# parrot-tts/Parrot-TTS

Hardware: AMD Instinct MI355X
Metric: audio samples/sec (16 kHz; see config.note) + RTF, 256-unit batch-64 per GPU (higher is better)
Workload: dtype f32 (f16x3 split products)

## Files before the change

### parrot_tts_amd/build.py

```python
from __future__ import annotations

import os
import subprocess
import sys
from concurrent.futures import ThreadPoolExecutor

HERE = os.path.dirname(os.path.abspath(__file__))
CSRC = os.path.join(HERE, "csrc")
LIB = os.path.join(HERE, "libparrot_hip.so")
OBJ = os.path.join(HERE, "build")
SOURCES = sorted(f for f in os.listdir(CSRC) if f.endswith(".hip"))
HEADERS = sorted(f for f in os.listdir(CSRC) if f.endswith(".h")) + [os.path.join("..", "..", "include", h) for h in ("parrot_hip.h", "parrot_hip_debug.h")]
FLAGS = ["--offload-arch=gfx950", "-O3", "-std=c++17", "-fPIC"]
TU_FLAGS = {f: ["-mllvm", "-disable-machine-sink"] for f in ("tu_split16.hip", "tu_split16_wide.hip", "tu_split16_xpl.hip")}


def _stale() -> bool:
    if not os.path.exists(LIB):
        return True
    t = os.path.getmtime(LIB)
    return any(os.path.getmtime(os.path.join(CSRC, f)) > t for f in SOURCES + HEADERS)


def build(force: bool = False, verbose: bool = False, extra_flags=(), lib_path: str = None, obj_dir: str = None) -> str:
    if lib_path is None and not force and not _stale():
        return LIB
    hipcc = os.environ.get("HIPCC", "/opt/rocm/bin/hipcc")
    LIB_OUT, OBJ_OUT = lib_path or LIB, obj_dir or OBJ
    os.makedirs(OBJ_OUT, exist_ok=True)

    def compile_one(src):
        obj = os.path.join(OBJ_OUT, os.path.splitext(src)[0] + ".o")
        tu = [] if os.environ.get("PARROT_NO_TU_FLAGS") else TU_FLAGS.get(src, [])
        cmd = [hipcc] + FLAGS + tu + list(extra_flags) + ["-c", os.path.join(CSRC, src), "-o", obj]
        if verbose:
            print(" ".join(cmd), file=sys.stderr)
        subprocess.run(cmd, check=True, cwd=CSRC)
# ... 21 lines not shown
```

### parrot_tts_amd/csrc/conv_mfma.h

```cpp
#pragma once
#include <hip/hip_runtime.h>
#include <stdint.h>
#include <algorithm>

#include "conv_consts.h"

namespace parrot {

__host__ __device__ __forceinline__ int row_true_len(int n, int mul, int add) { return n > 0 ? n * mul + add : 0; }

struct DynLdsOnce {
    bool done[64] = {};
};
inline hipError_t ensure_dyn_lds(DynLdsOnce& st, const void* kern, size_t lds) {
    int dev = 0;
    hipError_t e = hipGetDevice(&dev);
    if (e != hipSuccess) return e;
    const bool tracked = dev >= 0 && dev < 64;
    if (tracked && st.done[dev]) return hipSuccess;
    e = hipFuncSetAttribute(kern, hipFuncAttributeMaxDynamicSharedMemorySize, (int)lds);
    if (e == hipSuccess && tracked) st.done[dev] = true;
    return e;
}


typedef float f32x16 __attribute__((ext_vector_type(16)));
typedef float f32x4 __attribute__((ext_vector_type(4)));

// ... 145 lines not shown
            const int mbase = m_wave + mt * 32 + 4 * half;
            const int o0 = mbase / p.u, rem0 = mbase - o0 * p.u;
#pragma unroll
            for (int nt = 0; nt < WN; ++nt) {
                const int n = n_wave + nt * 32 + l31;
#pragma unroll
                for (int r = 0; r < 16; ++r) {
                    const int cr = (r & 3) + 8 * (r >> 2);
                    const int rem = rem0 + cr;
                    const int dq = (rem * p.u_inv16) >> 16;
                    const int o = o0 + dq;
                    const int tau = n * p.u + (rem - dq * p.u);
                    const bool ok = (mbase + cr < p.M) && (n < p.Ncols) && (tau < p.Tout);
                    const float v = acc[mt][nt][r] + ((p.bias && ok) ? p.bias[o] : 0.f);
                    if (ok) yb[o * p.Tout + tau] = apply_act(v, p.act);
                }
            }
        }
        return;
    }
    const bool late_res = rb != nullptr && !fold_res;
    const bool has_acc = p.epi != EPI_STORE;
    const bool do_div = p.epi == EPI_ADD_DIV;
    const float act_lo = (p.act == ACT_RELU) ? 0.f : -INFINITY;
#pragma unroll
    for (int mt = 0; mt < WM; ++mt) {
        const int mbase = m_wave + mt * 32 + 4 * half;
#pragma unroll
        for (int nt = 0; nt < WN; ++nt) {
            const int n = n_wave + nt * 32 + l31;
            const bool colok = n < p.Ncols;
#pragma unroll
            for (int g = 0; g < 2; ++g) {
                int off[8];
                float rv[8], yv[8];
#pragma unroll
                for (int q = 0; q < 8; ++q) {
                    const int r = g * 8 + q;
                    const int m = mbase + (r & 3) + 8 * (r >> 2);
                    off[q] = (colok && m < p.M) ? m * p.Tout + n : -1;
                    rv[q] = 0.f;
                    yv[q] = 0.f;
                }
                if (late_res) {
#pragma unroll
                    for (int q = 0; q < 8; ++q) rv[q] = rb[off[q] < 0 ? 0 : off[q]];
                }
                if (has_acc) {
#pragma unroll
                    for (int q = 0; q < 8; ++q) yv[q] = yb[off[q] < 0 ? 0 : off[q]];
                }
                float v[8];
#pragma unroll
                for (int q = 0; q < 8; ++q) v[q] = yv[q] + (fmaxf(acc[mt][nt][g * 8 + q], act_lo) + rv[q]);
                if (do_div) {
#pragma unroll
                    for (int q = 0; q < 8; ++q) v[q] = v[q] / p.div;
                }
#pragma unroll
                for (int q = 0; q < 8; ++q)
                    if (off[q] >= 0) yb[off[q]] = v[q];
            }
        }
    }
}

struct RowTile {
    __amdgpu_buffer_rsrc_t rsrc;
};
__device__ __forceinline__ RowTile row_tile(const float* base, int rows, int row_elems) {
    const size_t a = reinterpret_cast<size_t>(base);
    const unsigned lo = __builtin_amdgcn_readfirstlane((unsigned)a), hi = __builtin_amdgcn_readfirstlane((unsigned)(a >> 32));
    RowTile t;
    t.rsrc = __builtin_amdgcn_make_buffer_rsrc(reinterpret_cast<void*>(((size_t)hi << 32) | lo), 0,
                                               __builtin_amdgcn_readfirstlane(rows * row_elems * 4), 0x00020000);
    return t;
}
__device__ __forceinline__ float row_tile_load(const RowTile& t, int voff, int soff) {
    return __builtin_bit_cast(float, __builtin_amdgcn_raw_buffer_load_b32(t.rsrc, voff, soff, 0));
}
__device__ __forceinline__ void row_tile_store(const RowTile& t, float v, int voff, int soff) {
// ... 34 lines not shown
        for (int r = 0; r < 16; ++r) bs[r] = p.bias ? p.bias[min(m0 + 4 * half + (r & 3) + 8 * (r >> 2), p.M - 1)] * p.acc_scale : 0.f;
        if (fold_res) {
#pragma unroll
            for (int nt = 0; nt < WN; ++nt)
#pragma unroll
                for (int r = 0; r < 16; ++r) acc[mt][nt][r] = fmaf(acc[mt][nt][r], p.acc_scale, bs[r]);
        } else {
#pragma unroll
            for (int nt = 0; nt < WN; ++nt)
#pragma unroll
                for (int r = 0; r < 16; ++r) acc[mt][nt][r] = bs[r];
        }
    }
}

template <int WM, int WN>
__device__ __forceinline__ void conv_epilogue_lean(const ConvParams& p, f32x16 (&acc)[WM][WN], int b, int m_wave, int n_wave, int half, int l31) {
    float* __restrict__ yb = p.y + (size_t)b * p.y_bstride;
    const float* __restrict__ rb = p.res ? p.res + (size_t)b * p.res_bstride : nullptr;
    const bool fold_res = rb != nullptr && p.act == ACT_NONE && p.fold_res != 0;
    const bool late_res = rb != nullptr && !fold_res;
    const bool has_acc = p.epi != EPI_STORE;
    const bool do_div = p.epi == EPI_ADD_DIV;
    const bool relu = p.act == ACT_RELU;
    const int row_bytes = p.Tout * 4;
    int vo[WN];
#pragma unroll
    for (int nt = 0; nt < WN; ++nt) {
        const int n = n_wave + nt * 32 + l31;
        vo[nt] = (n < p.Ncols) ? (4 * half * p.Tout + n) * 4 : (int)0x80000000;
    }
    const RowTile yt = row_tile(yb, p.M, p.Tout), rt = row_tile(late_res ? rb : yb, p.M, p.Tout);
#pragma unroll
    for (int mt = 0; mt < WM; ++mt) {
        const int m0 = m_wave + mt * 32;
#pragma unroll
        for (int nt = 0; nt < WN; ++nt) {
            float v[16];
#pragma unroll
            for (int r = 0; r < 16; ++r) v[r] = acc[mt][nt][r] * p.out_scale;
            if (relu) {
#pragma unroll
                for (int r = 0; r < 16; ++r) v[r] = fmaxf(v[r], 0.f);
            }
            if (late_res) {
                float rv[16];
#pragma unroll
                for (int r = 0; r < 16; ++r) rv[r] = row_tile_load(rt, vo[nt], (m0 + (r & 3) + 8 * (r >> 2)) * row_bytes);
#pragma unroll
                for (int r = 0; r < 16; ++r) v[r] = v[r] + rv[r];
            }
            if (has_acc) {
                float yv[16];
#pragma unroll
                for (int r = 0; r < 16; ++r) yv[r] = row_tile_load(yt, vo[nt], (m0 + (r & 3) + 8 * (r >> 2)) * row_bytes);
#pragma unroll
                for (int r = 0; r < 16; ++r) v[r] = yv[r] + v[r];
                if (do_div) {
#pragma unroll
                    for (int r = 0; r < 16; ++r) v[r] = v[r] / p.div;
                }
            }
#pragma unroll
            for (int r = 0; r < 16; ++r) row_tile_store(yt, v[r], vo[nt], (m0 + (r & 3) + 8 * (r >> 2)) * row_bytes);
        }
    }
}

template <int WAVES_M, int WAVES_N, int WM, int WN, int CI, int MINW>
__global__ __launch_bounds__(WAVES_M* WAVES_N * 64, MINW) void conv_mfma_kernel(const ConvParams p) {
    constexpr int NW = WAVES_M * WAVES_N;
    constexpr int BM = WAVES_M * WM * 32;
    constexpr int BN = WAVES_N * WN * 32;
    constexpr int RS = BN + CONV_HALO;
    constexpr int QN = CI / 8;
    constexpr int ROWS_PW = CI / NW;
    constexpr int COLS_IT = (RS + 63) / 64;
    static_assert(CI % 8 == 0 && CI % NW == 0, "CI must be a multiple of 8 and of the wave count");

    extern __shared__ __attribute__((aligned(16))) float smem[];

    const int tid = threadIdx.x;
    const int lane = tid & 63;
    const int wave = __builtin_amdgcn_readfirstlane(tid >> 6);
// ... 156 lines not shown
```

### parrot_tts_amd/csrc/conv_mfma16.h

```cpp
#pragma once
#include "conv_mfma.h"

namespace parrot {

template <int NT16, int MINW>
__global__ __launch_bounds__(256, MINW) void conv_mfma16_kernel(const ConvParams p) {
    constexpr int WCOLS = NT16 * 16;
    constexpr int BN = 4 * WCOLS;
    constexpr int RS = BN + CONV_HALO + 16;
    constexpr int CI = 16;
    constexpr int ROWS_PW = CI / 4;
    constexpr int COLS_IT = (RS + 63) / 64;
    static_assert(RS % 32 == 16, "row stride must be 16 mod 32 dwords");

    extern __shared__ __attribute__((aligned(16))) float smem[];

    const int tid = threadIdx.x;
    const int lane = tid & 63;
    const int wave = __builtin_amdgcn_readfirstlane(tid >> 6);
    const int kg = lane >> 4;
    const int l15 = lane & 15;

    const int b = blockIdx.x / p.tiles_n;
    const int tn = blockIdx.x - b * p.tiles_n;
// ... 82 lines not shown
#pragma unroll
            for (int e = 0; e < 4; ++e)
#pragma unroll
                for (int nt = 0; nt < NT16; ++nt) bv_nxt[e][nt] = xn[(4 * e) * RS + nt * 16];
            __builtin_amdgcn_sched_barrier(0);
#pragma unroll
            for (int e = 0; e < 4; ++e)
#pragma unroll
                for (int nt = 0; nt < NT16; ++nt)
                    acc[nt] = __builtin_amdgcn_mfma_f32_16x16x4f32(a_cur[e], bv_cur[e][nt], acc[nt], 0, 0, 0);
            __builtin_amdgcn_sched_barrier(0);
#pragma unroll
            for (int e = 0; e < 4; ++e)
#pragma unroll
                for (int nt = 0; nt < NT16; ++nt) bv_cur[e][nt] = bv_nxt[e][nt];
        }
        if (more) store_slab((c + 1) & 1);
        __syncthreads();
    }

    const bool late_res = rb != nullptr && !fold_res;
    const bool has_acc = p.epi != EPI_STORE;
    const bool do_div = p.epi == EPI_ADD_DIV;
    const float act_lo = (p.act == ACT_RELU) ? 0.f : -INFINITY;
#pragma unroll
    for (int nt = 0; nt < NT16; ++nt) {
        const int n = n_wave + nt * 16 + l15;
        int off[4];
        float rv[4], yv[4], v[4];
#pragma unroll
        for (int r = 0; r < 4; ++r) {
            const int m = 4 * kg + r;
            off[r] = (n < p.Ncols && m < p.M) ? m * p.Tout + n : -1;
            rv[r] = 0.f;
            yv[r] = 0.f;
        }
        if (late_res) {
#pragma unroll
            for (int r = 0; r < 4; ++r) rv[r] = rb[off[r] < 0 ? 0 : off[r]];
        }
        if (has_acc) {
#pragma unroll
            for (int r = 0; r < 4; ++r) yv[r] = yb[off[r] < 0 ? 0 : off[r]];
        }
#pragma unroll
        for (int r = 0; r < 4; ++r) v[r] = yv[r] + (fmaxf(acc[nt][r], act_lo) + rv[r]);
        if (do_div) {
#pragma unroll
            for (int r = 0; r < 4; ++r) v[r] = v[r] / p.div;
        }
#pragma unroll
        for (int r = 0; r < 4; ++r)
            if (off[r] >= 0) yb[off[r]] = v[r];
    }
}

constexpr int MFMA16_NT16 = 8;
inline hipError_t launch_conv_mfma16(const ConvParams& p, hipStream_t s) {
    constexpr int BN = 4 * MFMA16_NT16 * 16;
    const size_t lds = (size_t)2 * 16 * (BN + CONV_HALO + 16) * sizeof(float);
    auto kern = conv_mfma16_kernel<MFMA16_NT16, 2>;
    static DynLdsOnce lds_once;
    {
        hipError_t e = ensure_dyn_lds(lds_once, reinterpret_cast<const void*>(kern), (size_t)lds);
        if (e != hipSuccess) return e;
    }
    hipLaunchKernelGGL(kern, dim3(p.tiles_n * p.B), dim3(256), lds, s, p);
    return hipGetLastError();
}

}
```

### parrot_tts_amd/csrc/conv_split16.h

```cpp
#pragma once
#include "conv_split.h"

#ifndef PARROT_XPL_DMA
#define PARROT_XPL_DMA 1
#endif

namespace parrot {

template <class SCH, int WAVES_M, int WAVES_N, int TM, int TN, int K, int MINW = 2, bool XPL = false>
__global__ __launch_bounds__(WAVES_M* WAVES_N * 64, MINW) void conv_split16_kernel(const ConvParams p) {
    static_assert(K > 0, "tap count is a template parameter");
    constexpr int NPC = SCH::NP, NTERM = SCH::NT;
    constexpr int NW = WAVES_M * WAVES_N, NT = NW * 64;
    constexpr int BM = WAVES_M * TM * 16, BN = WAVES_N * TN * 16;
    constexpr int COLS = (BN + CONV_HALO + 63) / 64 * 64;
    constexpr int OCT_BYTES = COLS * 16, PIECE_BYTES = 4 * OCT_BYTES, BUF_BYTES = NPC * PIECE_BYTES;
    constexpr int LIVE = COLS * 4;
    constexpr int ITEMS = (LIVE + NT - 1) / NT;
    constexpr int STEP_BYTES = NPC * 1024;
    static_assert(LIVE % NT == 0, "every thread stages the same number of items");

    extern __shared__ __attribute__((aligned(16))) char smem_raw[];

    const int tid = threadIdx.x;
// ... 174 lines not shown
#pragma unroll
                        for (int i = 0; i < NPC; ++i) __builtin_amdgcn_sched_group_barrier(0x100, 1, 0);
                    } else if (slab_left > 0) {
                        __builtin_amdgcn_sched_group_barrier(0x020, 1, 0);
                        --slab_left;
                    }
                }
#pragma unroll
                for (int i = 0; i < NPC; ++i) __builtin_amdgcn_sched_group_barrier(0x020, 1, 0);
            }
        }
        __builtin_amdgcn_sched_barrier(0);
        if (more) store_slab((c + 1) & 1);
        if constexpr (XPL && PARROT_XPL_DMA) asm volatile("s_waitcnt vmcnt(%0)" ::"n"(TM * NPC) : "memory");
        __syncthreads();
    }

    float* __restrict__ yb = p.y + (size_t)b * p.y_bstride;
    const float* __restrict__ rb = p.res ? p.res + (size_t)b * p.res_bstride : nullptr;
    const int out_row_bytes = p.Tout * 4;
    const bool late_res = rb != nullptr;
    const bool has_acc = p.epi != EPI_STORE;
    const bool do_div = p.epi == EPI_ADD_DIV;
    const bool relu = p.act == ACT_RELU;
    const RowTile yt = row_tile(yb, p.M, p.Tout), rt = row_tile(late_res ? rb : yb, p.M, p.Tout);
    if (p.yplane) {
        int vo[TN];
#pragma unroll
        for (int tn = 0; tn < TN; ++tn) {
            const int n = n_wave + tn * 16 + l15;
            vo[tn] = (n < p.Ncols) ? (4 * g4 * p.Tout + n) * 4 : (int)0x80000000;
        }
#pragma unroll
        for (int tm = 0; tm < TM; ++tm) {
            const int m0 = m_wave + tm * 16;
            float rv[TN][4];
            if (late_res) {
#pragma unroll
                for (int tn = 0; tn < TN; ++tn)
#pragma unroll
                    for (int r = 0; r < 4; ++r) rv[tn][r] = row_tile_load(rt, vo[tn], (m0 + r) * out_row_bytes);
            }
#pragma unroll
            for (int tn = 0; tn < TN; ++tn)
#pragma unroll
                for (int r = 0; r < 4; ++r) {
// ... 59 lines not shown
#pragma unroll
        for (int tm = 0; tm < TM; ++tm) {
            const int m0 = m_wave + tm * 16;
            const int soff = m0 * out_row_bytes;
            f32x4 rv[TN], yv[TN];
            if (late_res) {
#pragma unroll
                for (int q = 0; q < TN; ++q) rv[q] = row_tile_load4(rt, vq[q], soff);
            }
            if (has_acc) {
#pragma unroll
                for (int q = 0; q < TN; ++q) yv[q] = row_tile_load4(yt, vq[q], soff);
            }
#pragma unroll
            for (int tn = 0; tn < TN; ++tn)
#pragma unroll
                for (int r = 0; r < 4; ++r) {
                    float v = acc[tm][tn][r] * p.out_scale;
                    if (relu) v = fmaxf(v, 0.f);
                    stg[wbase + r * RS + tn * 16] = v;
                }
#pragma unroll
            for (int q = 0; q < TN; ++q) {
                f32x4 v = *reinterpret_cast<const f32x4*>(stg + lq[q]);
                if (late_res) v = v + rv[q];
                if (has_acc) {
                    v = yv[q] + v;
                    if (do_div) v = v / p.div;
                }
                row_tile_store4(yt, v, vq[q], soff);
            }
        }
        return;
    }
    int vo[TN];
#pragma unroll
    for (int tn = 0; tn < TN; ++tn) {
        const int n = n_wave + tn * 16 + l15;
        vo[tn] = (n < p.Ncols) ? (4 * g4 * p.Tout + n) * 4 : (int)0x80000000;
    }
#pragma unroll
    for (int tm = 0; tm < TM; ++tm) {
        const int m0 = m_wave + tm * 16;
        float v[TN][4];
#pragma unroll
        for (int tn = 0; tn < TN; ++tn)
#pragma unroll
            for (int r = 0; r < 4; ++r) v[tn][r] = acc[tm][tn][r] * p.out_scale;
        if (relu) {
#pragma unroll
            for (int tn = 0; tn < TN; ++tn)
#pragma unroll
                for (int r = 0; r < 4; ++r) v[tn][r] = fmaxf(v[tn][r], 0.f);
// ... 1 lines not shown
        if (late_res) {
            float rv[TN][4];
#pragma unroll
            for (int tn = 0; tn < TN; ++tn)
#pragma unroll
                for (int r = 0; r < 4; ++r) rv[tn][r] = row_tile_load(rt, vo[tn], (m0 + r) * out_row_bytes);
#pragma unroll
            for (int tn = 0; tn < TN; ++tn)
#pragma unroll
                for (int r = 0; r < 4; ++r) v[tn][r] = v[tn][r] + rv[tn][r];
        }
        if (has_acc) {
            float yv[TN][4];
#pragma unroll
            for (int tn = 0; tn < TN; ++tn)
#pragma unroll
                for (int r = 0; r < 4; ++r) yv[tn][r] = row_tile_load(yt, vo[tn], (m0 + r) * out_row_bytes);
#pragma unroll
            for (int tn = 0; tn < TN; ++tn)
#pragma unroll
                for (int r = 0; r < 4; ++r) v[tn][r] = yv[tn][r] + v[tn][r];
            if (do_div) {
#pragma unroll
                for (int tn = 0; tn < TN; ++tn)
#pragma unroll
                    for (int r = 0; r < 4; ++r) v[tn][r] = v[tn][r] / p.div;
            }
        }
#pragma unroll
        for (int tn = 0; tn < TN; ++tn)
#pragma unroll
            for (int r = 0; r < 4; ++r) row_tile_store(yt, v[tn][r], vo[tn], (m0 + r) * out_row_bytes);
    }
}

template <class SCH, int WAVES_M, int WAVES_N, int TM, int TN, int K, int MINW = 2, bool XPL = false>
inline hipError_t launch_conv_split16_t(const ConvParams& p, hipStream_t s) {
    constexpr int BM = WAVES_M * TM * 16, BN = WAVES_N * TN * 16, COLS = (BN + CONV_HALO + 63) / 64 * 64;
    const size_t lds = std::max((size_t)2 * SCH::NP * 4 * COLS * 16, (size_t)WAVES_M * WAVES_N * 16 * (TN * 16 + 4) * sizeof(float));
    auto kern = conv_split16_kernel<SCH, WAVES_M, WAVES_N, TM, TN, K, MINW, XPL>;
    static DynLdsOnce lds_once;
    {
        hipError_t e = ensure_dyn_lds(lds_once, reinterpret_cast<const void*>(kern), (size_t)lds);
        if (e != hipSuccess) return e;
    }
    const unsigned tiles = (unsigned)p.tiles_n * p.B, n_mb = (p.M + BM - 1) / BM;
    hipLaunchKernelGGL(kern, dim3((tiles + 7) / 8 * 8 * n_mb), dim3(WAVES_M * WAVES_N * 64), lds, s, p);
    return hipGetLastError();
}
// ... 88 lines not shown
```

### parrot_tts_amd/csrc/resblock_fused.h

```cpp
#pragma once
#include "conv_mfma.h"

namespace parrot {

constexpr int RB_MAX_CONVS = 8;
constexpr int RB_PAD = 32;

struct ResblockParams {
    const float* x;
    float* y;
    const float* wfrag[RB_MAX_CONVS];
    const float* bias[RB_MAX_CONVS];
    int dil[RB_MAX_CONVS];
    int n_conv;
    int type;
    int k, C, T, B;
    int H;
    int TT;
    int tiles;
    int epi;
    float div;
    float slope;
    const int32_t* row_len;
    int row_len_mul;
// ... 102 lines not shown
                }
            }
        }
    };

    float* cur = R;
    float* oth = S;
    if (p.type == 1) {
        for (int m = 0; m < p.n_conv; m += 2) {
            conv_phase(cur, oth, nullptr, p.wfrag[m], p.bias[m], p.dil[m], true, true);
            __syncthreads();
            conv_phase(oth, cur, cur, p.wfrag[m + 1], p.bias[m + 1], p.dil[m + 1], false, false);
            __syncthreads();
        }
    } else {
        for (int m = 0; m < p.n_conv; ++m) {
            conv_phase(cur, oth, cur, p.wfrag[m], p.bias[m], p.dil[m], true, false);
            __syncthreads();
            float* tmp = cur; cur = oth; oth = tmp;
        }
    }

    float* __restrict__ yb = p.y + (size_t)b * C * p.T;
    for (int idx = tid; idx < C * p.TT; idx += 512) {
        const int row = idx / p.TT, c = idx - row * p.TT;
        const int t = tile * p.TT + c;
        if (t < p.T) {
            float v = cur[row * RS + RB_PAD + p.H + c];
            const size_t o = (size_t)row * p.T + t;
            if (p.epi == EPI_ADD) v = yb[o] + v;
            else if (p.epi == EPI_ADD_DIV) v = (yb[o] + v) / p.div;
            yb[o] = v;
        }
    }
}

constexpr int RB16_PAD = 40;
static __global__ __launch_bounds__(512, 1) void resblock_fused16_kernel(const ResblockParams p) {
    constexpr int NT16 = 8;
    constexpr int W0 = 8 * NT16 * 16;
    constexpr int RS = W0 + 2 * RB16_PAD;
    static_assert(RS % 32 == 16, "row stride must be 16 mod 32 dwords");
    extern __shared__ __attribute__((aligned(16))) float smem[];

    const int tid = threadIdx.x;
    const int lane = tid & 63;
    const int wave = __builtin_amdgcn_readfirstlane(tid >> 6);
    const int kg = lane >> 4;
    const int l15 = lane & 15;
    const int b = blockIdx.x / p.tiles;
    const int tile = blockIdx.x - b * p.tiles;
    const int t_base = tile * p.TT - p.H;
    const int Tlim = p.row_len ? min(p.T, row_true_len(p.row_len[b], p.row_len_mul, p.row_len_add)) : p.T;
    constexpr int C = 16;
// ... 70 lines not shown
                v = (lrelu_out && v < 0.f) ? vs : v;
                dst[m * RS + RB16_PAD + c] = tok ? v : 0.f;
            }
        }
    };

    float* cur = R;
    float* oth = S;
    if (p.type == 1) {
        for (int m = 0; m < p.n_conv; m += 2) {
            conv_phase(cur, oth, nullptr, p.wfrag[m], p.bias[m], p.dil[m], true, true);
            __syncthreads();
            conv_phase(oth, cur, cur, p.wfrag[m + 1], p.bias[m + 1], p.dil[m + 1], false, false);
            __syncthreads();
        }
    } else {
        for (int m = 0; m < p.n_conv; ++m) {
            conv_phase(cur, oth, cur, p.wfrag[m], p.bias[m], p.dil[m], true, false);
            __syncthreads();
            float* tmp = cur; cur = oth; oth = tmp;
        }
    }
    float* __restrict__ yb = p.y + (size_t)b * C * p.T;
    for (int idx = tid; idx < C * p.TT; idx += 512) {
        const int row = idx / p.TT, c = idx - row * p.TT;
        const int t = tile * p.TT + c;
        if (t < p.T) {
            float v = cur[row * RS + RB16_PAD + p.H + c];
            const size_t o = (size_t)row * p.T + t;
            if (p.epi == EPI_ADD) v = yb[o] + v;
            else if (p.epi == EPI_ADD_DIV) v = (yb[o] + v) / p.div;
            yb[o] = v;
        }
    }
}

template <int NTW>
inline hipError_t launch_resblock_fused_t(const ResblockParams& p, hipStream_t s) {
    constexpr int RS = 8 * NTW * 32 + 2 * RB_PAD;
    const size_t lds = (size_t)2 * p.C * RS * sizeof(float);
    auto kern = resblock_fused_kernel<NTW>;
    static size_t attr_lds = 0;
    if (lds > attr_lds) {
        hipError_t e = hipFuncSetAttribute(reinterpret_cast<const void*>(kern), hipFuncAttributeMaxDynamicSharedMemorySize, (int)lds);
        if (e != hipSuccess) return e;
        attr_lds = lds;
    }
    hipLaunchKernelGGL(kern, dim3(p.tiles * p.B), dim3(512), lds, s, p);
    return hipGetLastError();
}

inline int resblock_window(int C) { return C <= 16 ? 1024 : 512; }
inline hipError_t launch_resblock_fused(const ResblockParams& p, hipStream_t s) {
    if (p.C == 16) {
// ... 14 lines not shown
```

### parrot_tts_amd/csrc/resblock_split.h

```cpp
#pragma once
#include "conv_split.h"

namespace parrot {

constexpr int RBS_MAX_CONVS = 8;
constexpr int RBS_MAX_BRANCH = 4;
constexpr int RBS_MAX_ALL = RBS_MAX_CONVS * RBS_MAX_BRANCH;

#ifdef RBS_TRACE
constexpr int RBS_TRACE_STAMPS = 128;
__device__ unsigned long long g_rbs_trace[8 * RBS_TRACE_STAMPS];
#define RBS_STAMP()                                                                                                   \
    do {                                                                                                              \
        if (trace_on && trace_n < RBS_TRACE_STAMPS) {                                                                 \
            const unsigned long long tt = __builtin_amdgcn_s_memtime();                                               \
            if (lane == 0) g_rbs_trace[wave * RBS_TRACE_STAMPS + trace_n] = tt;                                       \
        }                                                                                                             \
        ++trace_n;                                                                                                    \
    } while (0)
#else
#define RBS_STAMP() do {} while (0)
#endif
#ifndef RBS_EARLY_INNER
#define RBS_EARLY_INNER 1
#endif

struct ResblockSplitParams {
    const float* x;
    float* y;
    const uint16_t* wstream;
    const float* bias[RBS_MAX_ALL];
    float wsc[RBS_MAX_ALL];
    int dil[RBS_MAX_ALL];
    int n_conv;
    int k;
    int early;
    int n_branch;
    const uint16_t* bstream[RBS_MAX_BRANCH];
    int bk[RBS_MAX_BRANCH];
    int T, B;
    int H;
    int TT;
    int tiles;
    int epi;
    float div;
    float slope;
    const int32_t* row_len;
    int row_len_mul;
    int row_len_add;
};

constexpr int RBS_W = 384;

constexpr int rbs_default_wn(int nch) { return (nch / 2 >= 4) ? 1 : 4 / (nch / 2); }
template <class SCH, int NCH, int WN = 0, bool MRF = false>
__global__ __launch_bounds__((NCH / 2) * (WN ? WN : rbs_default_wn(NCH)) * 64,
                             ((NCH / 2) * (WN ? WN : rbs_default_wn(NCH)) * 64 == 512) ? 1 : (SCH::NP == 3 ? 2 : 3)) void resblock_split_kernel(const ResblockSplitParams p) {
    constexpr int NPC = SCH::NP, NTERM = SCH::NT, STEP_BYTES = SCH::NP * 1024;
    constexpr int C = 16 * NCH, WAVES_M = NCH / 2, WAVES_N = WN ? WN : rbs_default_wn(NCH), NTW = 3, W = WAVES_N * NTW * 32;
    const bool early = (WAVES_M == 1) && RBS_EARLY_INNER && __builtin_amdgcn_readfirstlane(p.early) != 0;
    int K = MRF ? p.bk[0] : p.k;
    constexpr int OCT_BYTES = W * 16, CH_BYTES = 2 * OCT_BYTES, PIECE_BYTES = NCH * CH_BYTES;
    static_assert(NCH == 2 || NCH == 4 || NCH == 8 || NCH == 16, "32, 64, 128 channels (4 waves: NCH / 2 row tiles x 4 / (NCH / 2) column groups) or 256 (8 waves)");
    extern __shared__ __attribute__((aligned(16))) char smem_raw[];

    const int tid = threadIdx.x;
    const int lane = tid & 63;
    const int wave = __builtin_amdgcn_readfirstlane(tid >> 6);
    const int wm = wave / WAVES_N;
    const int wn = wave % WAVES_N;
    const int half = lane >> 5;
    const int l31 = lane & 31;
    const int b = blockIdx.x / p.tiles;
    const int tile = blockIdx.x - b * p.tiles;
    const int t_base = tile * p.TT - p.H;
    const int Tlim = p.row_len ? min(p.T, row_true_len(p.row_len[b], p.row_len_mul, p.row_len_add)) : p.T;
    const bool edge = __builtin_amdgcn_readfirstlane((t_base < 0 || t_base + W > Tlim) ? 1 : 0);
#ifdef RBS_TRACE
    const bool trace_on = NCH == 2 && blockIdx.x == gridDim.x / 2;
    int trace_n = 0;
    RBS_STAMP();
#endif

    int col[NTW];
    bool tok[NTW];
#pragma unroll
    for (int nt = 0; nt < NTW; ++nt) {
        col[nt] = wn * (NTW * 32) + nt * 32 + l31;
        const int t = t_base + col[nt];
        tok[nt] = t >= 0 && t < Tlim;
    }

    f32x16 R[NTW], acc[NTW];
    auto load_r = [&]() __attribute__((always_inline)) {
        const size_t xaddr = reinterpret_cast<size_t>(p.x + (size_t)b * C * p.T);
        const unsigned x_lo = __builtin_amdgcn_readfirstlane((unsigned)xaddr), x_hi = __builtin_amdgcn_readfirstlane((unsigned)(xaddr >> 32));
        const __amdgpu_buffer_rsrc_t xrsrc =
            __builtin_amdgcn_make_buffer_rsrc(reinterpret_cast<void*>(((size_t)x_hi << 32) | x_lo), 0, 0x7fffffff, 0x00020000);
        const int row_bytes = p.T * 4;
#pragma unroll
        for (int nt = 0; nt < NTW; ++nt) {
            const int voff = tok[nt] ? (t_base + col[nt]) * 4 + 4 * half * row_bytes : (int)0x80000000;
#pragma unroll
            for (int r = 0; r < 16; ++r)
                R[nt][r] = __builtin_bit_cast(float, __builtin_amdgcn_raw_buffer_load_b32(xrsrc, voff, (32 * wm + (r & 3) + 8 * (r >> 2)) * row_bytes, 0));
        }
    };
    load_r();

    auto write_p = [&](const f32x16 (&v)[NTW], float mul, int part = 0) __attribute__((always_inline)) {
#pragma unroll
        for (int nt = 0; nt < NTW; ++nt) {
            if (part != 0 && (nt == 1) != (part == 1)) continue;
            const float m2 = (SCH::XS != 1.f) ? mul * p.slope : p.slope;
#pragma unroll
            for (int q = 0; q < 2; ++q) {
                unsigned qq[2][2][NPC];
#pragma unroll
                for (int g = 0; g < 2; ++g)
#pragma unroll
                    for (int e = 0; e < 2; ++e) {
                        const f32x2 vv = {v[nt][8 * q + 4 * g + 2 * e], v[nt][8 * q + 4 * g + 2 * e + 1]};
                        const f32x2 a = (SCH::XS != 1.f) ? vv * mul : vv, bq = vv * m2;
                        SCH::split(max_nc(a[0], bq[0]), max_nc(a[1], bq[1]), qq[g][e]);
                    }
                char* dst = smem_raw + (2 * wm + q) * CH_BYTES + half * OCT_BYTES + col[nt] * 16;
#pragma unroll
                for (int pc = 0; pc < NPC; ++pc) {
                    const auto r0 = __builtin_amdgcn_permlane32_swap(qq[0][0][pc], qq[1][0][pc], false, false);
                    const auto r1 = __builtin_amdgcn_permlane32_swap(qq[0][1][pc], qq[1][1][pc], false, false);
                    *reinterpret_cast<uint4*>(dst + pc * PIECE_BYTES) = uint4{r0[0], r1[0], r0[1], r1[1]};
                }
            }
        }
        if (edge) {
#pragma unroll
            for (int nt = 0; nt < NTW; ++nt)
                if (!tok[nt] && (part == 0 || (nt == 1) == (part == 1))) {
#pragma unroll
                    for (int q = 0; q < 2; ++q)
#pragma unroll
                        for (int pc = 0; pc < NPC; ++pc)
                            *reinterpret_cast<uint4*>(smem_raw + (2 * wm + q) * CH_BYTES + half * OCT_BYTES + col[nt] * 16 + pc * PIECE_BYTES) = uint4{0u, 0u, 0u, 0u};
                }
        }
    };

    auto stream_rsrc = [&](const uint16_t* ws) __attribute__((always_inline)) {
        const unsigned w_lo = __builtin_amdgcn_readfirstlane((unsigned)reinterpret_cast<size_t>(ws));
        const unsigned w_hi = __builtin_amdgcn_readfirstlane((unsigned)(reinterpret_cast<size_t>(ws) >> 32));
        return __builtin_amdgcn_make_buffer_rsrc(reinterpret_cast<void*>(((size_t)w_hi << 32) | w_lo), 0, 0x7fffffff, 0x00020000);
    };
    __amdgpu_buffer_rsrc_t wrsrc = stream_rsrc(MRF ? p.bstream[0] : p.wstream);
    const unsigned lane16 = lane * 16;
    s16x8 A[2][NPC], Bv[2][NTW][NPC];
    auto load_a_piece = [&](s16x8 (&a)[NPC], int pc, int gstep) __attribute__((always_inline)) {
        a[pc] = __builtin_bit_cast(s16x8, __builtin_amdgcn_raw_buffer_load_b128(wrsrc, lane16 + pc * 1024, gstep * STEP_BYTES, 0));
    };
    int conv_steps = WAVES_M * NCH * K;
    int gbase = wm * NCH * K;
#pragma unroll
    for (int pc = 0; pc < NPC; ++pc) {
        load_a_piece(A[0], pc, gbase);
        load_a_piece(A[1], pc, gbase + K);
    }

    RBS_STAMP();
    write_p(R, SCH::XS);
    RBS_STAMP();
    __syncthreads();
    RBS_STAMP();

    int center = (K - 1) / 2;
    auto load_b = [&](s16x8 (&bb)[NTW][NPC], int ch, int shift) __attribute__((always_inline)) {
#pragma unroll
        for (int nt = 0; nt < NTW; ++nt) {
            const char* src = smem_raw + ch * CH_BYTES + half * OCT_BYTES + (col[nt] + shift) * 16;
#pragma unroll
            for (int pc = 0; pc < NPC; ++pc) bb[nt][pc] = *reinterpret_cast<const s16x8*>(src + pc * PIECE_BYTES);
        }
    };
    auto conv = [&](f32x16 (&acc)[NTW], int dil) __attribute__((always_inline)) {
        load_b(Bv[0], 0, -center * dil);
        for (int j = 0; j < K; ++j) {
            const int shift = (j - center) * dil;
            const int n0 = (j + 1 < K) ? gbase + j + 1 : gbase + conv_steps;
#pragma unroll
            for (int ch = 0; ch < NCH; ++ch) {
                const int set = ch & 1;
                if (ch + 1 < NCH) load_b(Bv[set ^ 1], ch + 1, shift);
                else load_b(Bv[set ^ 1], 0, shift + dil);
                const int nx = (ch + 2 < NCH) ? gbase + (ch + 2) * K + j : n0 + (ch + 2 - NCH) * K;
#pragma unroll
                for (int t = 0; t < NTERM; ++t) {
#pragma unroll
                    for (int nt = 0; nt < NTW; ++nt) acc[nt] = mfma32<SCH>(A[set][SCH::pa(t)], Bv[set][nt][SCH::pb(t)], acc[nt]);
#pragma unroll
                    for (int pc = 0; pc < NPC; ++pc)
                        if (t == SCH::last_a(pc)) load_a_piece(A[set], pc, nx);
                }
// ... 98 lines not shown
            RBS_STAMP();
        }
    }
    if constexpr (SCH::XS != 1.f) {
        const float inv = 1.f / rs;
#pragma unroll
        for (int nt = 0; nt < NTW; ++nt)
#pragma unroll
            for (int r = 0; r < 16; ++r) R[nt][r] = R[nt][r] * inv;
    }
    if constexpr (MRF) {
#pragma unroll
        for (int nt = 0; nt < NTW; ++nt)
#pragma unroll
            for (int r = 0; r < 16; ++r) XSr[nt][r] = (br == 0) ? 0.f + R[nt][r] : XSr[nt][r] + R[nt][r];
    }
    }

    RBS_STAMP();
    const RowTile yt = row_tile(p.y + (size_t)b * C * p.T, C, p.T);
    const int row_bytes = p.T * 4;
    const bool has_acc = !MRF && p.epi != EPI_STORE;
    const bool do_div = p.epi == EPI_ADD_DIV;
#pragma unroll
    for (int nt = 0; nt < NTW; ++nt) {
        const int c = col[nt] - p.H;
        const int t = tile * p.TT + c;
        const bool ok = c >= 0 && c < p.TT && t < p.T;
        const int voff = ok ? (4 * half * p.T + t) * 4 : (int)0x80000000;
        float v[16];
        if constexpr (MRF) {
#pragma unroll
            for (int r = 0; r < 16; ++r) v[r] = (n_branch > 1) ? XSr[nt][r] / p.div : XSr[nt][r];
        } else if (has_acc) {
            float yv[16];
#pragma unroll
            for (int r = 0; r < 16; ++r) yv[r] = row_tile_load(yt, voff, (32 * wm + (r & 3) + 8 * (r >> 2)) * row_bytes);
#pragma unroll
            for (int r = 0; r < 16; ++r) v[r] = yv[r] + R[nt][r];
            if (do_div) {
#pragma unroll
                for (int r = 0; r < 16; ++r) v[r] = v[r] / p.div;
            }
        } else {
#pragma unroll
            for (int r = 0; r < 16; ++r) v[r] = 0.f + R[nt][r];
        }
#pragma unroll
        for (int r = 0; r < 16; ++r) row_tile_store(yt, v[r], voff, (32 * wm + (r & 3) + 8 * (r >> 2)) * row_bytes);
    }
}

constexpr int RBS16_W = 768;

template <class SCH>
__global__ __launch_bounds__(256, SCH::NP == 3 ? 2 : 3) void resblock16_split_kernel(const ResblockSplitParams p) {
    constexpr int NPC = SCH::NP, NTERM = SCH::NT, STEP_BYTES = SCH::NP * 1024;
    constexpr int C = 16, NT = 12, W = RBS16_W, NP = NT / 2;
    const int K = p.k, S = (K + 1) / 2;
    constexpr int OCT_BYTES = W * 16, PIECE_BYTES = 2 * OCT_BYTES;
    static_assert(4 * NT * 16 == W, "4 waves x NT tiles cover the window");
    extern __shared__ __attribute__((aligned(16))) char smem_raw[];

    const int tid = threadIdx.x;
    const int lane = tid & 63;
    const int wave = __builtin_amdgcn_readfirstlane(tid >> 6);
// ... 12 lines not shown
        const size_t xaddr = reinterpret_cast<size_t>(p.x + (size_t)b * C * p.T);
        const unsigned x_lo = __builtin_amdgcn_readfirstlane((unsigned)xaddr), x_hi = __builtin_amdgcn_readfirstlane((unsigned)(xaddr >> 32));
        const __amdgpu_buffer_rsrc_t xrsrc =
            __builtin_amdgcn_make_buffer_rsrc(reinterpret_cast<void*>(((size_t)x_hi << 32) | x_lo), 0, 0x7fffffff, 0x00020000);
        const int row_bytes = p.T * 4;
#pragma unroll
        for (int nt = 0; nt < NT; ++nt) {
            const int t = t_base + col0 + nt * 16;
            const int voff = (t >= 0 && t < Tlim) ? t * 4 + 4 * g4 * row_bytes : (int)0x80000000;
#pragma unroll
            for (int r = 0; r < 4; ++r) R[nt][r] = __builtin_bit_cast(float, __builtin_amdgcn_raw_buffer_load_b32(xrsrc, voff, r * row_bytes, 0));
        }
    }
    auto write_p = [&](const f32x4 (&v)[NT], float mul, int part = 0) __attribute__((always_inline)) {
        const float m2 = (SCH::XS != 1.f) ? mul * p.slope : p.slope;
#pragma unroll
        for (int np = 0; np < NT; np += 2) {
            if (part != 0 && (np >= 2 && np < NT - 2) != (part == 1)) continue;
            unsigned qq[2][2][NPC];
#pragma unroll
            for (int u = 0; u < 2; ++u) {
#pragma unroll
                for (int e = 0; e < 2; ++e) {
                    const f32x2 vv = {v[np + u][2 * e], v[np + u][2 * e + 1]};
                    const f32x2 a = (SCH::XS != 1.f) ? vv * mul : vv, bq = vv * m2;
                    SCH::split(max_nc(a[0], bq[0]), max_nc(a[1], bq[1]), qq[u][e]);
                }
            }
            const int c = col0 + (np + (g4 & 1)) * 16;
            char* dst = smem_raw + (g4 >> 1) * OCT_BYTES + c * 16;
#pragma unroll
            for (int pc = 0; pc < NPC; ++pc) {
                const auto r0 = __builtin_amdgcn_permlane16_swap(qq[0][0][pc], qq[1][0][pc], false, false);
                const auto r1 = __builtin_amdgcn_permlane16_swap(qq[0][1][pc], qq[1][1][pc], false, false);
                *reinterpret_cast<uint4*>(dst + pc * PIECE_BYTES) = uint4{r0[0], r1[0], r0[1], r1[1]};
            }
        }
        if (edge) {
#pragma unroll
            for (int np = 0; np < NT; np += 2) {
                if (part != 0 && (np >= 2 && np < NT - 2) != (part == 1)) continue;
                const int c = col0 + (np + (g4 & 1)) * 16;
                const int t = t_base + c;
                if (!(t >= 0 && t < Tlim)) {
#pragma unroll
                    for (int pc = 0; pc < NPC; ++pc)
                        *reinterpret_cast<uint4*>(smem_raw + (g4 >> 1) * OCT_BYTES + c * 16 + pc * PIECE_BYTES) = uint4{0u, 0u, 0u, 0u};
                }
            }
// ... 89 lines not shown
        for (int r = 0; r < 4; ++r) bv[r] = p.bias[m + 1][4 * g4 + r];
#pragma unroll
        for (int nt = 0; nt < NT; ++nt)
#pragma unroll
            for (int r = 0; r < 4; ++r) acc[nt][r] = (SCH::XS != 1.f) ? bv[r] * s2 : bv[r];
        conv(p.dil[m + 1]);
        const float i2 = 1.f / s2;
#pragma unroll
        for (int nt = 0; nt < NT; ++nt)
#pragma unroll
            for (int r = 0; r < 4; ++r) R[nt][r] = (SCH::XS != 1.f) ? fmaf(acc[nt][r], i2, R[nt][r]) : acc[nt][r] + R[nt][r];
        if (m + 2 < p.n_conv) {
            if (early) write_p(R, SCH::XS, 1);
            __syncthreads();
            write_p(R, SCH::XS, early ? 2 : 0);
            __syncthreads();
        }
    }

    const RowTile yt = row_tile(p.y + (size_t)b * C * p.T, C, p.T);
    const int row_bytes = p.T * 4;
    const bool has_acc = p.epi != EPI_STORE;
    const bool do_div = p.epi == EPI_ADD_DIV;
    if (has_acc) {
#pragma unroll
        for (int n0 = 0; n0 < NT; n0 += 4) {
            float yv[4][4];
            int voff[4];
#pragma unroll
            for (int i = 0; i < 4; ++i) {
                const int c = col0 + (n0 + i) * 16 - p.H;
                const int t = tile * p.TT + c;
                voff[i] = (c >= 0 && c < p.TT && t < p.T) ? (4 * g4 * p.T + t) * 4 : (int)0x80000000;
#pragma unroll
                for (int r = 0; r < 4; ++r) yv[i][r] = row_tile_load(yt, voff[i], r * row_bytes);
            }
#pragma unroll
            for (int i = 0; i < 4; ++i)
#pragma unroll
                for (int r = 0; r < 4; ++r) {
                    float v = yv[i][r] + R[n0 + i][r];
                    if (do_div) v = v / p.div;
                    row_tile_store(yt, v, voff[i], r * row_bytes);
                }
        }
    } else {
#pragma unroll
        for (int nt = 0; nt < NT; ++nt) {
            const int c = col0 + nt * 16 - p.H;
            const int t = tile * p.TT + c;
            const int voff = (c >= 0 && c < p.TT && t < p.T) ? (4 * g4 * p.T + t) * 4 : (int)0x80000000;
#pragma unroll
            for (int r = 0; r < 4; ++r) row_tile_store(yt, 0.f + R[nt][r], voff, r * row_bytes);
        }
    }
}

template <class SCH>
inline hipError_t launch_resblock_split_s(int C, const ResblockSplitParams& p, hipStream_t s) {
    const size_t lds = (size_t)SCH::NP * 2 * RBS_W * 32 * (C == 256 ? 2 : 1);
    auto kern = (C == 16) ? resblock16_split_kernel<SCH> : (C == 256) ? resblock_split_kernel<SCH, 16> : (C == 128) ? resblock_split_kernel<SCH, 8>
              : (C == 64) ? resblock_split_kernel<SCH, 4> : resblock_split_kernel<SCH, 2>;
    static DynLdsOnce lds_once[5];
    const int slot = (C == 16) ? 0 : (C == 256) ? 4 : (C == 128) ? 3 : (C == 64) ? 2 : 1;
    {
        hipError_t e = ensure_dyn_lds(lds_once[slot], reinterpret_cast<const void*>(kern), lds);
        if (e != hipSuccess) return e;
// ... 54 lines not shown
```

Before: 297.3 million.

## Replace uniform float division with reciprocal or FMA paths and tune resblock codegen

Adds a DivUniform helper that, once per kernel, sorts the epilogue divisor into three cases. Power-of-two divisors become a multiply by the reciprocal, a divisor of 3 uses a corrected reciprocal-FMA, and anything else keeps true division. All conv and resblock epilogues now use it instead of per-element IEEE divides. Separately it disables SLP vectorization for several translation units, turns the f32x2 vector ops in the split-packing code into scalar ops, replaces per-tile column arrays with one base pointer plus fixed offsets, and adds an occupancy knob for the NCH==2 resblock variant. The divide change must stay bit-exact with true division for the divisors it covers, and the codegen changes may shift register pressure either way.

```diff
diff --git a/parrot_tts_amd/build.py b/parrot_tts_amd/build.py
--- a/parrot_tts_amd/build.py
+++ b/parrot_tts_amd/build.py
@@ -13,6 +13,11 @@
 HEADERS = sorted(f for f in os.listdir(CSRC) if f.endswith(".h")) + [os.path.join("..", "..", "include", h) for h in ("parrot_hip.h", "parrot_hip_debug.h")]
 FLAGS = ["--offload-arch=gfx950", "-O3", "-std=c++17", "-fPIC"]
 TU_FLAGS = {f: ["-mllvm", "-disable-machine-sink"] for f in ("tu_split16.hip", "tu_split16_wide.hip", "tu_split16_xpl.hip")}
+NO_SLP_UNITS = ("tu_mrf.hip", "tu_mrf_single.hip", "tu_resblock.hip", "tu_split16.hip", "tu_split16_single.hip",
+                "tu_split16_single_f16.hip", "tu_split16_wide.hip", "tu_split16_xpl.hip", "tu_split_bf16x6.hip", "tu_split_f16x3.hip",
+                "tu_split_single.hip", "tu_attn.hip")
+for _f in NO_SLP_UNITS:
+    TU_FLAGS[_f] = TU_FLAGS.get(_f, []) + ["-fno-slp-vectorize"]
 
 
 def _stale() -> bool:
diff --git a/parrot_tts_amd/csrc/conv_mfma.h b/parrot_tts_amd/csrc/conv_mfma.h
--- a/parrot_tts_amd/csrc/conv_mfma.h
+++ b/parrot_tts_amd/csrc/conv_mfma.h
@@ -4,6 +4,7 @@
 #include <algorithm>
 
 #include "conv_consts.h"
+#include "div_uniform.h"
 
 namespace parrot {
 
@@ -195,6 +196,7 @@
     const bool late_res = rb != nullptr && !fold_res;
     const bool has_acc = p.epi != EPI_STORE;
     const bool do_div = p.epi == EPI_ADD_DIV;
+    const DivUniform dv = div_uniform(p.div);
     const float act_lo = (p.act == ACT_RELU) ? 0.f : -INFINITY;
 #pragma unroll
     for (int mt = 0; mt < WM; ++mt) {
@@ -226,10 +228,7 @@
                 float v[8];
 #pragma unroll
                 for (int q = 0; q < 8; ++q) v[q] = yv[q] + (fmaxf(acc[mt][nt][g * 8 + q], act_lo) + rv[q]);
-                if (do_div) {
-#pragma unroll
-                    for (int q = 0; q < 8; ++q) v[q] = v[q] / p.div;
-                }
+                if (do_div) div_rows(dv, v);
 #pragma unroll
                 for (int q = 0; q < 8; ++q)
                     if (off[q] >= 0) yb[off[q]] = v[q];
@@ -310,6 +309,7 @@
     const bool late_res = rb != nullptr && !fold_res;
     const bool has_acc = p.epi != EPI_STORE;
     const bool do_div = p.epi == EPI_ADD_DIV;
+    const DivUniform dv = div_uniform(p.div);
     const bool relu = p.act == ACT_RELU;
     const int row_bytes = p.Tout * 4;
     int vo[WN];
@@ -344,10 +344,7 @@
                 for (int r = 0; r < 16; ++r) yv[r] = row_tile_load(yt, vo[nt], (m0 + (r & 3) + 8 * (r >> 2)) * row_bytes);
 #pragma unroll
                 for (int r = 0; r < 16; ++r) v[r] = yv[r] + v[r];
-                if (do_div) {
-#pragma unroll
-                    for (int r = 0; r < 16; ++r) v[r] = v[r] / p.div;
-                }
+                if (do_div) div_rows(dv, v);
             }
 #pragma unroll
             for (int r = 0; r < 16; ++r) row_tile_store(yt, v[r], vo[nt], (m0 + (r & 3) + 8 * (r >> 2)) * row_bytes);
diff --git a/parrot_tts_amd/csrc/conv_mfma16.h b/parrot_tts_amd/csrc/conv_mfma16.h
--- a/parrot_tts_amd/csrc/conv_mfma16.h
+++ b/parrot_tts_amd/csrc/conv_mfma16.h
@@ -128,6 +128,7 @@
     const bool late_res = rb != nullptr && !fold_res;
     const bool has_acc = p.epi != EPI_STORE;
     const bool do_div = p.epi == EPI_ADD_DIV;
+    const DivUniform dv = div_uniform(p.div);
     const float act_lo = (p.act == ACT_RELU) ? 0.f : -INFINITY;
 #pragma unroll
     for (int nt = 0; nt < NT16; ++nt) {
@@ -151,10 +152,7 @@
         }
 #pragma unroll
         for (int r = 0; r < 4; ++r) v[r] = yv[r] + (fmaxf(acc[nt][r], act_lo) + rv[r]);
-        if (do_div) {
-#pragma unroll
-            for (int r = 0; r < 4; ++r) v[r] = v[r] / p.div;
-        }
+        if (do_div) div_rows(dv, v);
 #pragma unroll
         for (int r = 0; r < 4; ++r)
             if (off[r] >= 0) yb[off[r]] = v[r];
diff --git a/parrot_tts_amd/csrc/conv_split16.h b/parrot_tts_amd/csrc/conv_split16.h
--- a/parrot_tts_amd/csrc/conv_split16.h
+++ b/parrot_tts_amd/csrc/conv_split16.h
@@ -220,6 +220,7 @@
     const bool late_res = rb != nullptr;
     const bool has_acc = p.epi != EPI_STORE;
     const bool do_div = p.epi == EPI_ADD_DIV;
+    const DivUniform dv = div_uniform(p.div);
     const bool relu = p.act == ACT_RELU;
     const RowTile yt = row_tile(yb, p.M, p.Tout), rt = row_tile(late_res ? rb : yb, p.M, p.Tout);
     if (p.yplane) {
@@ -325,13 +326,16 @@
                 }
 #pragma unroll
             for (int q = 0; q < TN; ++q) {
-                f32x4 v = *reinterpret_cast<const f32x4*>(stg + lq[q]);
-                if (late_res) v = v + rv[q];
+                const f32x4 sv = *reinterpret_cast<const f32x4*>(stg + lq[q]);
+                float v[4];
+#pragma unroll
+                for (int e = 0; e < 4; ++e) v[e] = late_res ? sv[e] + rv[q][e] : sv[e];
                 if (has_acc) {
-                    v = yv[q] + v;
-                    if (do_div) v = v / p.div;
-                }
-                row_tile_store4(yt, v, vq[q], soff);
+#pragma unroll
+                    for (int e = 0; e < 4; ++e) v[e] = yv[q][e] + v[e];
+                    if (do_div) div_rows(dv, v);
+                }
+                row_tile_store4(yt, f32x4{v[0], v[1], v[2], v[3]}, vq[q], soff);
             }
         }
         return;
@@ -379,9 +383,7 @@
                 for (int r = 0; r < 4; ++r) v[tn][r] = yv[tn][r] + v[tn][r];
             if (do_div) {
 #pragma unroll
-                for (int tn = 0; tn < TN; ++tn)
-#pragma unroll
-                    for (int r = 0; r < 4; ++r) v[tn][r] = v[tn][r] / p.div;
+                for (int tn = 0; tn < TN; ++tn) div_rows(dv, v[tn]);
             }
         }
 #pragma unroll
diff --git a/parrot_tts_amd/csrc/div_uniform.h b/parrot_tts_amd/csrc/div_uniform.h
--- /dev/null
+++ b/parrot_tts_amd/csrc/div_uniform.h
@@ -0,0 +1,63 @@
+#pragma once
+#include <cmath>
+#include <cstdint>
+#include <cstring>
+
+#if defined(__HIPCC__)
+#define PARROT_HD __host__ __device__ __forceinline__
+#else
+#define PARROT_HD inline
+#endif
+
+namespace parrot {
+
+enum { DIV_TRUE = 0, DIV_MUL = 1, DIV_FMA3 = 2 };
+
+struct DivUniform {
+    float d, r;
+    int mode;
+};
+
+PARROT_HD DivUniform div_uniform(float d) {
+    DivUniform u;
+    u.d = d;
+    u.r = 1.f / d;
+    uint32_t bits;
+#if defined(__HIP_DEVICE_COMPILE__)
+    bits = __builtin_bit_cast(uint32_t, d);
+#else
+    std::memcpy(&bits, &d, 4);
+#endif
+    const uint32_t ex = (bits >> 23) & 0xff;
+    const bool pow2 = (bits & 0x007fffffu) == 0 && ex >= 1 && ex <= 253;
+    u.mode = pow2 ? DIV_MUL : (d == 3.f ? DIV_FMA3 : DIV_TRUE);
+    return u;
+}
+
+PARROT_HD float div3_fma(float x, float d, float r) {
+    const float q = x * r;
+    const float e = __builtin_fmaf(-q, d, x);
+    return (e < 0.f || e > 0.f) ? __builtin_fmaf(e, r, q) : q;
+}
+
+PARROT_HD float div_apply(const DivUniform& u, float x) {
+    if (u.mode == DIV_FMA3) return div3_fma(x, u.d, u.r);
+    if (u.mode == DIV_MUL) return x * u.r;
+    return x / u.d;
+}
+
+template <int N>
+PARROT_HD void div_rows(const DivUniform& u, float (&v)[N]) {
+    if (u.mode == DIV_FMA3) {
+#pragma unroll
+        for (int i = 0; i < N; ++i) v[i] = div3_fma(v[i], u.d, u.r);
+    } else if (u.mode == DIV_MUL) {
+#pragma unroll
+        for (int i = 0; i < N; ++i) v[i] = v[i] * u.r;
+    } else {
+#pragma unroll
+        for (int i = 0; i < N; ++i) v[i] = v[i] / u.d;
+    }
+}
+
+}
diff --git a/parrot_tts_amd/csrc/resblock_fused.h b/parrot_tts_amd/csrc/resblock_fused.h
--- a/parrot_tts_amd/csrc/resblock_fused.h
+++ b/parrot_tts_amd/csrc/resblock_fused.h
@@ -148,6 +148,7 @@
     }
 
     float* __restrict__ yb = p.y + (size_t)b * C * p.T;
+    const DivUniform dv = div_uniform(p.div);
     for (int idx = tid; idx < C * p.TT; idx += 512) {
         const int row = idx / p.TT, c = idx - row * p.TT;
         const int t = tile * p.TT + c;
@@ -155,7 +156,7 @@
             float v = cur[row * RS + RB_PAD + p.H + c];
             const size_t o = (size_t)row * p.T + t;
             if (p.epi == EPI_ADD) v = yb[o] + v;
-            else if (p.epi == EPI_ADD_DIV) v = (yb[o] + v) / p.div;
+            else if (p.epi == EPI_ADD_DIV) v = div_apply(dv, yb[o] + v);
             yb[o] = v;
         }
     }
@@ -272,6 +273,7 @@
         }
     }
     float* __restrict__ yb = p.y + (size_t)b * C * p.T;
+    const DivUniform dv = div_uniform(p.div);
     for (int idx = tid; idx < C * p.TT; idx += 512) {
         const int row = idx / p.TT, c = idx - row * p.TT;
         const int t = tile * p.TT + c;
@@ -279,7 +281,7 @@
             float v = cur[row * RS + RB16_PAD + p.H + c];
             const size_t o = (size_t)row * p.T + t;
             if (p.epi == EPI_ADD) v = yb[o] + v;
-            else if (p.epi == EPI_ADD_DIV) v = (yb[o] + v) / p.div;
+            else if (p.epi == EPI_ADD_DIV) v = div_apply(dv, yb[o] + v);
             yb[o] = v;
         }
     }
diff --git a/parrot_tts_amd/csrc/resblock_split.h b/parrot_tts_amd/csrc/resblock_split.h
--- a/parrot_tts_amd/csrc/resblock_split.h
+++ b/parrot_tts_amd/csrc/resblock_split.h
@@ -23,6 +23,9 @@
 #endif
 #ifndef RBS_EARLY_INNER
 #define RBS_EARLY_INNER 1
+#endif
+#ifndef RBS_WG_32
+#define RBS_WG_32 3
 #endif
 
 struct ResblockSplitParams {
@@ -55,7 +58,7 @@
 constexpr int rbs_default_wn(int nch) { return (nch / 2 >= 4) ? 1 : 4 / (nch / 2); }
 template <class SCH, int NCH, int WN = 0, bool MRF = false>
 __global__ __launch_bounds__((NCH / 2) * (WN ? WN : rbs_default_wn(NCH)) * 64,
-                             ((NCH / 2) * (WN ? WN : rbs_default_wn(NCH)) * 64 == 512) ? 1 : (SCH::NP == 3 ? 2 : 3)) void resblock_split_kernel(const ResblockSplitParams p) {
+                             ((NCH / 2) * (WN ? WN : rbs_default_wn(NCH)) * 64 == 512) ? 1 : (SCH::NP == 3 ? 2 : (NCH == 2 ? RBS_WG_32 : 3))) void resblock_split_kernel(const ResblockSplitParams p) {
     constexpr int NPC = SCH::NP, NTERM = SCH::NT, STEP_BYTES = SCH::NP * 1024;
     constexpr int C = 16 * NCH, WAVES_M = NCH / 2, WAVES_N = WN ? WN : rbs_default_wn(NCH), NTW = 3, W = WAVES_N * NTW * 32;
     const bool early = (WAVES_M == 1) && RBS_EARLY_INNER && __builtin_amdgcn_readfirstlane(p.early) != 0;
@@ -82,12 +85,13 @@
     RBS_STAMP();
 #endif
 
-    int col[NTW];
+    const int col0 = wn * (NTW * 32) + l31;
+    char* const slot0 = smem_raw + half * OCT_BYTES + col0 * 16;
+    auto colf = [&](int nt) __attribute__((always_inline)) { return col0 + nt * 32; };
     bool tok[NTW];
 #pragma unroll
     for (int nt = 0; nt < NTW; ++nt) {
-        col[nt] = wn * (NTW * 32) + nt * 32 + l31;
-        const int t = t_base + col[nt];
+        const int t = t_base + colf(nt);
         tok[nt] = t >= 0 && t < Tlim;
     }
 
@@ -100,7 +104,7 @@
         const int row_bytes = p.T * 4;
 #pragma unroll
         for (int nt = 0; nt < NTW; ++nt) {
-            const int voff = tok[nt] ? (t_base + col[nt]) * 4 + 4 * half * row_bytes : (int)0x80000000;
+            const int voff = tok[nt] ? (t_base + colf(nt)) * 4 + 4 * half * row_bytes : (int)0x80000000;
 #pragma unroll
             for (int r = 0; r < 16; ++r)
                 R[nt][r] = __builtin_bit_cast(float, __builtin_amdgcn_raw_buffer_load_b32(xrsrc, voff, (32 * wm + (r & 3) + 8 * (r >> 2)) * row_bytes, 0));
@@ -120,11 +124,11 @@
                 for (int g = 0; g < 2; ++g)
 #pragma unroll
                     for (int e = 0; e < 2; ++e) {
-                        const f32x2 vv = {v[nt][8 * q + 4 * g + 2 * e], v[nt][8 * q + 4 * g + 2 * e + 1]};
-                        const f32x2 a = (SCH::XS != 1.f) ? vv * mul : vv, bq = vv * m2;
-                        SCH::split(max_nc(a[0], bq[0]), max_nc(a[1], bq[1]), qq[g][e]);
+                        const float v0 = v[nt][8 * q + 4 * g + 2 * e], v1 = v[nt][8 * q + 4 * g + 2 * e + 1];
+                        const float a0 = (SCH::XS != 1.f) ? v0 * mul : v0, a1 = (SCH::XS != 1.f) ? v1 * mul : v1;
+                        SCH::split(max_nc(a0, v0 * m2), max_nc(a1, v1 * m2), qq[g][e]);
                     }
-                char* dst = smem_raw + (2 * wm + q) * CH_BYTES + half * OCT_BYTES + col[nt] * 16;
+                char* dst = slot0 + (2 * wm + q) * CH_BYTES + nt * 512;
 #pragma unroll
                 for (int pc = 0; pc < NPC; ++pc) {
                     const auto r0 = __builtin_amdgcn_permlane32_swap(qq[0][0][pc], qq[1][0][pc], false, false);
@@ -141,7 +145,7 @@
                     for (int q = 0; q < 2; ++q)
 #pragma unroll
                         for (int pc = 0; pc < NPC; ++pc)
-                            *reinterpret_cast<uint4*>(smem_raw + (2 * wm + q) * CH_BYTES + half * OCT_BYTES + col[nt] * 16 + pc * PIECE_BYTES) = uint4{0u, 0u, 0u, 0u};
+                            *reinterpret_cast<uint4*>(slot0 + (2 * wm + q) * CH_BYTES + nt * 512 + pc * PIECE_BYTES) = uint4{0u, 0u, 0u, 0u};
                 }
         }
     };
@@ -175,7 +179,7 @@
     auto load_b = [&](s16x8 (&bb)[NTW][NPC], int ch, int shift) __attribute__((always_inline)) {
 #pragma unroll
         for (int nt = 0; nt < NTW; ++nt) {
-            const char* src = smem_raw + ch * CH_BYTES + half * OCT_BYTES + (col[nt] + shift) * 16;
+            const char* src = slot0 + shift * 16 + ch * CH_BYTES + nt * 512;
 #pragma unroll
             for (int pc = 0; pc < NPC; ++pc) bb[nt][pc] = *reinterpret_cast<const s16x8*>(src + pc * PIECE_BYTES);
         }
@@ -320,26 +324,25 @@
     const int row_bytes = p.T * 4;
     const bool has_acc = !MRF && p.epi != EPI_STORE;
     const bool do_div = p.epi == EPI_ADD_DIV;
+    const DivUniform dv = div_uniform(p.div);
 #pragma unroll
     for (int nt = 0; nt < NTW; ++nt) {
-        const int c = col[nt] - p.H;
+        const int c = colf(nt) - p.H;
         const int t = tile * p.TT + c;
         const bool ok = c >= 0 && c < p.TT && t < p.T;
         const int voff = ok ? (4 * half * p.T + t) * 4 : (int)0x80000000;
         float v[16];
         if constexpr (MRF) {
 #pragma unroll
-            for (int r = 0; r < 16; ++r) v[r] = (n_branch > 1) ? XSr[nt][r] / p.div : XSr[nt][r];
+            for (int r = 0; r < 16; ++r) v[r] = XSr[nt][r];
+            if (n_branch > 1) div_rows(dv, v);
         } else if (has_acc) {
             float yv[16];
 #pragma unroll
             for (int r = 0; r < 16; ++r) yv[r] = row_tile_load(yt, voff, (32 * wm + (r & 3) + 8 * (r >> 2)) * row_bytes);
 #pragma unroll
             for (int r = 0; r < 16; ++r) v[r] = yv[r] + R[nt][r];
-            if (do_div) {
-#pragma unroll
-                for (int r = 0; r < 16; ++r) v[r] = v[r] / p.div;
-            }
+            if (do_div) div_rows(dv, v);
         } else {
 #pragma unroll
             for (int r = 0; r < 16; ++r) v[r] = 0.f + R[nt][r];
@@ -398,9 +401,9 @@
             for (int u = 0; u < 2; ++u) {
 #pragma unroll
                 for (int e = 0; e < 2; ++e) {
-                    const f32x2 vv = {v[np + u][2 * e], v[np + u][2 * e + 1]};
-                    const f32x2 a = (SCH::XS != 1.f) ? vv * mul : vv, bq = vv * m2;
-                    SCH::split(max_nc(a[0], bq[0]), max_nc(a[1], bq[1]), qq[u][e]);
+                    const float v0 = v[np + u][2 * e], v1 = v[np + u][2 * e + 1];
+                    const float a0 = (SCH::XS != 1.f) ? v0 * mul : v0, a1 = (SCH::XS != 1.f) ? v1 * mul : v1;
+                    SCH::split(max_nc(a0, v0 * m2), max_nc(a1, v1 * m2), qq[u][e]);
                 }
             }
             const int c = col0 + (np + (g4 & 1)) * 16;
@@ -536,6 +539,7 @@
     const int row_bytes = p.T * 4;
     const bool has_acc = p.epi != EPI_STORE;
     const bool do_div = p.epi == EPI_ADD_DIV;
+    const DivUniform dv = div_uniform(p.div);
     if (has_acc) {
 #pragma unroll
         for (int n0 = 0; n0 < NT; n0 += 4) {
@@ -550,13 +554,14 @@
                 for (int r = 0; r < 4; ++r) yv[i][r] = row_tile_load(yt, voff[i], r * row_bytes);
             }
 #pragma unroll
-            for (int i = 0; i < 4; ++i)
-#pragma unroll
-                for (int r = 0; r < 4; ++r) {
-                    float v = yv[i][r] + R[n0 + i][r];
-                    if (do_div) v = v / p.div;
-                    row_tile_store(yt, v, voff[i], r * row_bytes);
-                }
+            for (int i = 0; i < 4; ++i) {
+                float v[4];
+#pragma unroll
+                for (int r = 0; r < 4; ++r) v[r] = yv[i][r] + R[n0 + i][r];
+                if (do_div) div_rows(dv, v);
+#pragma unroll
+                for (int r = 0; r < 4; ++r) row_tile_store(yt, v[r], voff[i], r * row_bytes);
+            }
         }
     } else {
 #pragma unroll
```

After: 302.8 million (median of 6 runs). 1.9% higher.
